# flyakon/DeepPhysiNet

Hardware: AMD Instinct MI355X
Metric: collocation-points/sec (fwd+PDE-Jacobian+bwd) (higher is better)
Workload: dtype bf16x2 (hi+lo split bf16 MFMA operands), fp32 accumulate

## Files before the change

deepphysinet_amd/csrc/dpn_device.h:

```cpp
#pragma once
#include <hip/hip_runtime.h>
#include <stdint.h>
#include <stdio.h>
#include <stdlib.h>

#include "../../include/dpn_hip.h"
#include "dpn_layout.h"

using namespace dpn;

typedef __attribute__((ext_vector_type(8))) __bf16 bf16x8;
typedef __attribute__((ext_vector_type(16))) float f32x16;
typedef unsigned short u16;

#define DEV __device__ __forceinline__

typedef unsigned int u32;
typedef __attribute__((ext_vector_type(2))) __bf16 bf16x2;
typedef __attribute__((ext_vector_type(2))) float f32x2;
typedef __attribute__((ext_vector_type(4))) u32 u32x4;
typedef __attribute__((ext_vector_type(4))) float f32x4;

DEV u32 pack2(float a, float b) {
    const f32x2 v = {a, b};
    return __builtin_bit_cast(u32, __builtin_convertvector(v, bf16x2));
}
DEV float bf_lo(u32 w) { return __uint_as_float(w << 16); }
DEV float bf_hi(u32 w) { return __uint_as_float(w & 0xFFFF0000u); }

DEV bf16x8 as_bf(u32x4 w) { return __builtin_bit_cast(bf16x8, w); }
DEV f32x16 mfma(bf16x8 a, bf16x8 b, f32x16 c) { return __builtin_amdgcn_mfma_f32_32x32x16_bf16(a, b, c, 0, 0, 0); }

static inline int ck(hipError_t e) { return (int)e; }
```

deepphysinet_amd/csrc/dpn_encoder_chain.hip:

```cpp
#include <atomic>
#include <hip/hip_runtime.h>
#include <stdint.h>
#include <stdlib.h>

#include "../../include/dpn_hip.h"
#include "../../include/dpn_hip_experiments.h"

#define DEV __device__ __forceinline__

namespace {

typedef _Float16 f16x8 __attribute__((ext_vector_type(8)));
typedef float f32x4 __attribute__((ext_vector_type(4)));
typedef unsigned int u32;
typedef u32 u32x4 __attribute__((ext_vector_type(4)));

constexpr int kD = 256;
constexpr int kThreads = 512, kWaves = 8;
constexpr int kImgBytes = 256 * 1024;
#ifndef DPN_ENC_PF
#define DPN_ENC_PF 8
#endif
template <int NTT> constexpr int pf_of() { return NTT == 1 ? DPN_ENC_PF : 4; }
constexpr int kYS = 260;
constexpr int kXImg = 16384;
constexpr float kLoScale = 2048.0f, kLoInv = 1.0f / 2048.0f;

#ifdef DPN_ENC_TIMELINE
unsigned* g_enc_timeline = nullptr;
#define ENC_STAMP(I) do { if (a.tl && lane == 0) a.tl[((size_t)tl_block * kWaves + wave) * 32 + (I)] = (unsigned)__builtin_readcyclecounter(); } while (0)
#define ENC_TL_ARG unsigned* tl;
#define ENC_TL_SET(A) (A).tl = g_enc_timeline
#else
#define ENC_STAMP(I) do { } while (0)
#define ENC_TL_ARG
#define ENC_TL_SET(A) do { } while (0)
#endif

DEV void barrier_lds() {
    __builtin_amdgcn_fence(__ATOMIC_RELEASE, "workgroup", "local");
    __builtin_amdgcn_s_barrier();
    __builtin_amdgcn_fence(__ATOMIC_ACQUIRE, "workgroup", "local");
}

template <int CTRL>
DEV float dpp(float v) { return __builtin_bit_cast(float, __builtin_amdgcn_update_dpp(0, __builtin_bit_cast(int, v), CTRL, 0xf, 0xf, false)); }
DEV float swz16(float v) { return __builtin_bit_cast(float, __builtin_amdgcn_ds_swizzle(__builtin_bit_cast(int, v), 0x401F)); }
DEV float half_sum(float v) {
    v += dpp<0xB1>(v);
    v += dpp<0x4E>(v);
    v += dpp<0x141>(v);
    v += dpp<0x140>(v);
    v += swz16(v);
    return v;
}
DEV float half_max(float v) {
    v = fmaxf(v, dpp<0xB1>(v));
    v = fmaxf(v, dpp<0x4E>(v));
    v = fmaxf(v, dpp<0x141>(v));
    v = fmaxf(v, dpp<0x140>(v));
    v = fmaxf(v, swz16(v));
    return v;
}

DEV float gelu_exact(float x) { return x * 0.5f * (1.0f + erff(x * 0.70710678118654752440f)); }
DEV float gelu_exact_grad(float x) {
    const float cdf = 0.5f * (1.0f + erff(x * 0.70710678118654752440f));
    const float pdf = expf(-0.5f * x * x) * 0.39894228040143267794f;
    return cdf + x * pdf;
}

DEV void split8(const float (&v)[8], u32x4& hi, u32x4& lo) {
    f16x8 h, l;
#pragma unroll
    for (int e = 0; e < 8; ++e) {
        const _Float16 a = (_Float16)v[e];
        h[e] = a;
        l[e] = (_Float16)((v[e] - (float)a) * kLoScale);
    }
    hi = __builtin_bit_cast(u32x4, h);
    lo = __builtin_bit_cast(u32x4, l);
}

DEV int xpos(int slot, int n) { return slot * 16 + (n ^ ((slot & 3) | ((slot & 4) ? 12 : 0))); }

struct RowLane {
    int tsel, slot, n16;
    DEV RowLane(int wave, int lane) : tsel(lane >> 5), slot(lane & 31), n16(2 * wave + (lane >> 5)) {}
};

DEV void row_to_ximg(const float (&v)[8], const float extra_max, const RowLane& rl, char* ximg_tile, float* rscale_tile) {
    float m = extra_max;
#pragma unroll
    for (int e = 0; e < 8; ++e) m = fmaxf(m, fabsf(v[e]));
    m = half_max(m);
    int eb = (__builtin_bit_cast(int, m) >> 23) & 0xff;
    eb = eb < 4 ? 4 : eb;
    const float sc = __builtin_bit_cast(float, (257 - eb) << 23);
    float s[8];
#pragma unroll
    for (int e = 0; e < 8; ++e) s[e] = v[e] * sc;
    u32x4 hi, lo;
    split8(s, hi, lo);
    char* p = ximg_tile + xpos(rl.slot, rl.n16) * 16;
    *reinterpret_cast<u32x4*>(p) = hi;
    *reinterpret_cast<u32x4*>(p + kXImg / 2) = lo;
    if (rl.slot == 0) rscale_tile[rl.n16] = __builtin_bit_cast(float, (eb - 3) << 23);
}
DEV float row_absmax(const float (&v)[8]) {
    float m = 0.f;
#pragma unroll
    for (int e = 0; e < 8; ++e) m = fmaxf(m, fabsf(v[e]));
    return m;
}

DEV void load8(float (&v)[8], const float* p, bool ok) {
    if (ok) {
        const float4 a = reinterpret_cast<const float4*>(p)[0], b = reinterpret_cast<const float4*>(p)[1];
        v[0] = a.x; v[1] = a.y; v[2] = a.z; v[3] = a.w; v[4] = b.x; v[5] = b.y; v[6] = b.z; v[7] = b.w;
    } else {
#pragma unroll
        for (int e = 0; e < 8; ++e) v[e] = 0.f;
    }
}
DEV void store8(float* p, const float (&v)[8], bool ok) {
    if (ok) {
        reinterpret_cast<float4*>(p)[0] = make_float4(v[0], v[1], v[2], v[3]);
        reinterpret_cast<float4*>(p)[1] = make_float4(v[4], v[5], v[6], v[7]);
    }
}
DEV void lds8(float (&v)[8], const float* p) {
    const f32x4 a = reinterpret_cast<const f32x4*>(p)[0], b = reinterpret_cast<const f32x4*>(p)[1];
    v[0] = a[0]; v[1] = a[1]; v[2] = a[2]; v[3] = a[3]; v[4] = b[0]; v[5] = b[1]; v[6] = b[2]; v[7] = b[3];
}

DEV void layer_norm8(const float (&v)[8], const float (&gam)[8], const float (&bet)[8], float (&xhat)[8], float (&y)[8], float& rstd) {
    float s = 0.f;
#pragma unroll
    for (int e = 0; e < 8; ++e) s += v[e];
    const float mean = half_sum(s) * (1.f / kD);
    float d[8], q = 0.f;
#pragma unroll
    for (int e = 0; e < 8; ++e) { d[e] = v[e] - mean; q = fmaf(d[e], d[e], q); }
    rstd = 1.0f / sqrtf(half_sum(q) * (1.f / kD) + 1e-5f);
#pragma unroll
    for (int e = 0; e < 8; ++e) { xhat[e] = d[e] * rstd; y[e] = fmaf(xhat[e], gam[e], bet[e]); }
}
DEV void layer_norm_bwd8(const float (&g)[8], const float (&xhat)[8], const float rstd, const float (&gam)[8], float (&gx)[8], float (&pg)[8],
                         float (&pb)[8]) {
    float t[8], s1 = 0.f, s2 = 0.f;
#pragma unroll
    for (int e = 0; e < 8; ++e) { t[e] = g[e] * gam[e]; s1 += t[e]; s2 = fmaf(t[e], xhat[e], s2); pg[e] = fmaf(g[e], xhat[e], pg[e]); pb[e] += g[e]; }
    const float m1 = half_sum(s1) * (1.f / kD), m2 = half_sum(s2) * (1.f / kD);
#pragma unroll
    for (int e = 0; e < 8; ++e) gx[e] = rstd * (t[e] - m1 - xhat[e] * m2);
}

struct WStream {
    __amdgpu_buffer_rsrc_t rs;
    int voff, tile_off;
    DEV void init(const void* wpack, int64_t bytes, int wave, int lane) {
        rs = __builtin_amdgcn_make_buffer_rsrc(const_cast<void*>(wpack), 0, (int)bytes, 0x00020000);
        voff = lane * 16;
        tile_off = wave * 2 * 16384;
    }
    template <int NT>
    DEV void load(u32x4 (&dst)[NT][2], int img_off, int ks) const {
#pragma unroll
        for (int t = 0; t < NT; ++t)
#pragma unroll
            for (int p = 0; p < 2; ++p)
                dst[t][p] = __builtin_bit_cast(u32x4, __builtin_amdgcn_raw_buffer_load_b128(rs, voff + p * 1024, img_off + tile_off + t * 16384 + ks * 2048, 0));
    }
};
template <int PF, int NT = 2> struct Ring { u32x4 a[PF][NT][2]; };

DEV f32x4 mfma(u32x4 a, u32x4 b, f32x4 c) {
    return __builtin_amdgcn_mfma_f32_16x16x32_f16(__builtin_bit_cast(f16x8, a), __builtin_bit_cast(f16x8, b), c, 0, 0, 0);
}

template <int NTT, int NT = 2>
struct Acc {
    f32x4 m[NT][NTT], c[NT][NTT];
    DEV void zero() {
#pragma unroll
        for (int t = 0; t < NT; ++t)
#pragma unroll
            for (int tt = 0; tt < NTT; ++tt) { m[t][tt] = (f32x4)0.f; c[t][tt] = (f32x4)0.f; }
    }
};

template <int NTT, bool HAS_NEXT, int NT = 2>
DEV void gemm(const WStream& ws, Ring<pf_of<NTT>(), NT>& R, const int cur_off, const int next_off, const char* xr0, const char* xr1, Acc<NTT, NT>& acc) {
    u32x4 B[2][NTT][2];
    auto loadB = [&](const int ks, const int buf) __attribute__((always_inline)) {
        const char* base = ((ks & 1) ? xr1 : xr0) + ks * 1024;
// ... 1320 lines not shown
```

deepphysinet_amd/csrc/dpn_fwd_tiles.h:

```cpp
#pragma once

namespace ts {
constexpr int kVecFloats = kNumVecs * 256 + 4;
template <int NS>
struct Cfg {
    static constexpr int kXBytes = 16 * 2 * NS * 1024;
    static constexpr int kVecOff = kXBytes;
    static constexpr int kRedOff = kVecOff + kVecFloats * 4;
    static constexpr int kLdsBytes = kRedOff + 4 * 64 * 4;
};

DEV void barrier_lds() {
    __builtin_amdgcn_fence(__ATOMIC_RELEASE, "workgroup", "local");
    __builtin_amdgcn_s_barrier();
    __builtin_amdgcn_fence(__ATOMIC_ACQUIRE, "workgroup", "local");
}

struct NoSide { DEV void operator()(int) const {} };

#ifdef TS_ABL_NOSINCOS
template <int NS> DEV void ts_sincos(float th, float& s, float& c) { s = th; c = th * 0.5f; }
#else
template <int NS> DEV void ts_sincos(float th, float& s, float& c) { sincos_t<NS>(th, s, c); }
#endif

template <int NS, bool SWAP = false>
DEV void mma3(const u32x4 (&a)[NS], const u32x4 (&b)[NS], f32x16& acc) {
#ifdef TS_ABL_NOMFMA
    if constexpr (NS == 2) asm volatile("" ::"v"(a[0]), "v"(a[1]), "v"(b[0]), "v"(b[1]));
    else asm volatile("" ::"v"(a[0]), "v"(b[0]));
    return;
#endif
    if constexpr (SWAP) {
        if constexpr (NS == 2) {
            acc = mfma(as_bf(b[1]), as_bf(a[0]), acc);
            acc = mfma(as_bf(b[0]), as_bf(a[1]), acc);
        }
        acc = mfma(as_bf(b[0]), as_bf(a[0]), acc);
    } else {
        if constexpr (NS == 2) {
            acc = mfma(as_bf(a[0]), as_bf(b[1]), acc);
            acc = mfma(as_bf(a[1]), as_bf(b[0]), acc);
        }
        acc = mfma(as_bf(a[0]), as_bf(b[0]), acc);
    }
}

#ifndef TS_PF
#define TS_PF 3
#endif
#ifndef TS_PRIO
#define TS_PRIO 2
#endif
#ifndef TS_DEFER_SAVES
#define TS_DEFER_SAVES 1
#endif
#ifndef TS_SCHED_GROUPS
#define TS_SCHED_GROUPS 0
#endif
constexpr int kPF = TS_PF;
template <int NS, int NT> struct Head { u32x4 a[kPF - 1][NT][NS]; };

template <int NS, int NK, int NT>
struct WSrc {
    __amdgpu_buffer_rsrc_t rs;
    int voff;
    int so[NT];
    DEV void init(const char* wg, const int lane, const int ks0) {
        rs = __builtin_amdgcn_make_buffer_rsrc(const_cast<char*>(wg), 0, NT * NK * NS * 1024, 0x00020000);
        voff = lane * 16;
#pragma unroll
        for (int t = 0; t < NT; ++t) { so[t] = (t * NK + ks0) * NS * 1024; asm volatile("" : "+s"(so[t])); }
    }
    DEV void next(u32x4 (&dst)[NT][NS]) {
#pragma unroll
        for (int t = 0; t < NT; ++t) {
#pragma unroll
            for (int s = 0; s < NS; ++s) {
#ifdef TS_ABL_NOALOAD
                asm volatile("" : "=v"(dst[t][s]));
#else
                dst[t][s] = __builtin_bit_cast(u32x4, __builtin_amdgcn_raw_buffer_load_b128(rs, voff + s * 1024, so[t], 0));
#endif
            }
            so[t] += NS * 1024;
            asm volatile("" : "+s"(so[t]));
        }
    }
};
template <int NS, int NK, int NT>
DEV void gemm_head(const char* wg, const int lane, Head<NS, NT>& H) {
    WSrc<NS, NK, NT> src;
    src.init(wg, lane, 0);
#pragma unroll
    for (int k = 0; k < kPF - 1; ++k) src.next(H.a[k]);
}
template <int NS, int NK, int NT, bool SWAP = false, class Side = NoSide, bool PIN = true, bool SG = PIN>
DEV void gemm(const char* wg, const char* xl, const int lane, const Head<NS, NT>& H, f32x16 (&acc)[2][2], const Side& side = Side()) {
    static_assert(NK >= kPF, "k-steps per chunk");
    WSrc<NS, NK, NT> src;
    src.init(wg, lane, kPF - 1);
    u32x4 A[kPF][NT][NS];
    u32x4 B[2][2][NS];
    auto loadB = [&](const int ks, const int slot) __attribute__((always_inline)) {
#pragma unroll
        for (int p = 0; p < 2; ++p)
#pragma unroll
            for (int s = 0; s < NS; ++s) B[slot][p][s] = *reinterpret_cast<const u32x4*>(xl + ((ks * 2 + p) * NS + s) * 1024);
    };
#pragma unroll
    for (int k = 0; k < kPF - 1; ++k)
#pragma unroll
        for (int t = 0; t < NT; ++t)
#pragma unroll
            for (int s = 0; s < NS; ++s) A[k][t][s] = H.a[k][t][s];
    loadB(0, 0);
#if TS_PRIO == 2
    __builtin_amdgcn_s_setprio(0);
#endif
#pragma unroll
    for (int ks = 0; ks < NK; ++ks) {
        if (ks + kPF - 1 < NK) src.next(A[(ks + kPF - 1) % kPF]);
        if (ks + 1 < NK) loadB(ks + 1, (ks + 1) & 1);
#if TS_SCHED_GROUPS
        if (SG && ks + 1 < NK) {
            __builtin_amdgcn_sched_group_barrier(0x100, 2 * NS, 0);
            __builtin_amdgcn_sched_group_barrier(0x008, 4 * (NS == 2 ? 3 : 1), 0);
        }
#endif
#if TS_PRIO == 1
        __builtin_amdgcn_s_setprio(1);
#endif
#pragma unroll
        for (int t = 0; t < NT; ++t)
#pragma unroll
            for (int p = 0; p < 2; ++p) mma3<NS, SWAP>(A[ks % kPF][t], B[ks & 1][p], acc[t][p]);
#if TS_PRIO == 1
        __builtin_amdgcn_s_setprio(0);
#endif
        side(ks);
        if constexpr (PIN) {
        asm volatile("" : "+v"(acc[0][0]), "+v"(acc[0][1]), "+v"(acc[1][0]), "+v"(acc[1][1]));
        }
    }
#if TS_PRIO == 2
    __builtin_amdgcn_s_setprio(1);
#endif
}

template <int NS>
DEV void x_store(char* xl, const int ks, const int p, const Frag<NS>& f) {
#pragma unroll
    for (int s = 0; s < NS; ++s) *reinterpret_cast<u32x4*>(xl + ((ks * 2 + p) * NS + s) * 1024) = f.w[s];
}

DEV void acc_init(f32x16& acc, const float* vec, const int which, const int h, const int T, const float scale) {
    const f32x4* v = reinterpret_cast<const f32x4*>(vec + which * 256 + h * 128 + T * 16);
#pragma unroll
    for (int q = 0; q < 4; ++q) {
        const f32x4 x = v[q];
        acc[4 * q] = scale * x[0]; acc[4 * q + 1] = scale * x[1]; acc[4 * q + 2] = scale * x[2]; acc[4 * q + 3] = scale * x[3];
    }
}

struct Ident { u32x4 a, b; };
DEV Ident make_ident(const int j, const int h) {
    Ident I;
    const int mine = (((j >> 3) & 1) == h) ? (j & 7) : -1;
#pragma unroll
// ... 138 lines not shown
```

deepphysinet_amd/csrc/dpn_gemm.hip:

```cpp
#include "dpn_device.h"

struct SgemmArgs {
    const float *A, *B, *bias;
    float *C, *asum, *ws;
    int M, N, K, lda, ldb, ldc, ta, tb, accumulate, k_per_split;
};

__global__ __launch_bounds__(256) void dpn_sgemm_kernel(SgemmArgs a) {
    constexpr int BM = 32, BN = 32, BK = 32;
    __shared__ float As[BK][BM + 1];
    __shared__ float Bs[BK][BN + 1];
    const int tx = threadIdx.x & 15, ty = threadIdx.x >> 4;
    const int m0 = blockIdx.y * BM, n0 = blockIdx.x * BN;
    const int kbeg = blockIdx.z * a.k_per_split;
    const int kend = (kbeg + a.k_per_split < a.K) ? kbeg + a.k_per_split : a.K;
    const bool split = gridDim.z > 1;
    float acc[2][2] = {{0.f, 0.f}, {0.f, 0.f}};
    float rs = 0.f;
    const bool do_asum = a.asum != nullptr && blockIdx.x == 0;
    float ra[4], rb[4];
    auto gload = [&](int k0) __attribute__((always_inline)) {
#pragma unroll
        for (int i = 0; i < 4; ++i) {
            const int e = threadIdx.x + 256 * i;
            {
                const int kk = a.ta ? (e >> 5) : (e & 31), mm = a.ta ? (e & 31) : (e >> 5);
                const int gm = m0 + mm, gk = k0 + kk;
                ra[i] = (gm < a.M && gk < kend) ? (a.ta ? a.A[(int64_t)gk * a.lda + gm] : a.A[(int64_t)gm * a.lda + gk]) : 0.f;
            }
            {
                const int kk = a.tb ? (e & 31) : (e >> 5), nn = a.tb ? (e >> 5) : (e & 31);
                const int gk = k0 + kk, gn = n0 + nn;
                rb[i] = (gk < kend && gn < a.N) ? (a.tb ? a.B[(int64_t)gn * a.ldb + gk] : a.B[(int64_t)gk * a.ldb + gn]) : 0.f;
            }
        }
    };
    gload(kbeg);
    for (int k0 = kbeg; k0 < kend; k0 += BK) {
#pragma unroll
        for (int i = 0; i < 4; ++i) {
            const int e = threadIdx.x + 256 * i;
            As[a.ta ? (e >> 5) : (e & 31)][a.ta ? (e & 31) : (e >> 5)] = ra[i];
            Bs[a.tb ? (e & 31) : (e >> 5)][a.tb ? (e >> 5) : (e & 31)] = rb[i];
        }
        __syncthreads();
        if (k0 + BK < kend) gload(k0 + BK);
#pragma unroll
        for (int kk = 0; kk < BK; ++kk) {
            const float a0 = As[kk][ty], a1 = As[kk][ty + 16], b0 = Bs[kk][tx], b1 = Bs[kk][tx + 16];
            acc[0][0] = fmaf(a0, b0, acc[0][0]); acc[0][1] = fmaf(a0, b1, acc[0][1]);
            acc[1][0] = fmaf(a1, b0, acc[1][0]); acc[1][1] = fmaf(a1, b1, acc[1][1]);
        }
        if (do_asum && threadIdx.x < BM) {
#pragma unroll
            for (int kk = 0; kk < BK; ++kk) rs += As[kk][threadIdx.x];
        }
        __syncthreads();
    }
#pragma unroll
    for (int i = 0; i < 2; ++i)
#pragma unroll
        for (int j = 0; j < 2; ++j) {
            const int gm = m0 + ty + 16 * i, gn = n0 + tx + 16 * j;
            if (gm < a.M && gn < a.N) {
                if (split) {
                    a.ws[((int64_t)blockIdx.z * a.M + gm) * a.N + gn] = acc[i][j];
                } else {
                    const float v = acc[i][j] + (a.bias ? a.bias[gn] : 0.f);
                    float* c = a.C + (int64_t)gm * a.ldc + gn;
                    *c = a.accumulate ? (*c + v) : v;
                }
            }
        }
    if (do_asum && threadIdx.x < BM && m0 + threadIdx.x < a.M) {
        if (split) a.ws[(int64_t)gridDim.z * a.M * a.N + (int64_t)blockIdx.z * a.M + m0 + threadIdx.x] = rs;
        else a.asum[m0 + threadIdx.x] = rs;
    }
}

__global__ __launch_bounds__(256) void dpn_sgemm_reduce_kernel(SgemmArgs a, int splits) {
    const int64_t idx = (int64_t)blockIdx.x * 256 + threadIdx.x;
    const int64_t mn = (int64_t)a.M * a.N;
    if (idx < mn) {
        float v = 0.f;
        for (int z = 0; z < splits; ++z) v += a.ws[z * mn + idx];
        const int gm = (int)(idx / a.N), gn = (int)(idx % a.N);
        v += a.bias ? a.bias[gn] : 0.f;
        float* c = a.C + (int64_t)gm * a.ldc + gn;
        *c = a.accumulate ? (*c + v) : v;
    }
    if (a.asum && idx < a.M) {
        float v = 0.f;
        for (int z = 0; z < splits; ++z) v += a.ws[splits * mn + (int64_t)z * a.M + idx];
        a.asum[idx] = v;
    }
}

constexpr int kBatchMaxProblems = DPN_GEMM_MAX_PROBLEMS, kBatchMaxTerms = DPN_GEMM_MAX_TERMS, kBatchTermPool = 32, kBatchMaxJobs = DPN_GEMM_MAX_JOBS;
struct SgemmTerm {
    const float* A;
    const float* B;
    int lda, ldb, K, pad;
};
struct SgemmProblem {
    const float* bias;
    float *C, *asum;
    const float* aux;
    float* aux_out;
    int M, N, ldc, ta, tb, nterms, term0, epi;
};
DEV float gelu_exact(float x) { return x * 0.5f * (1.0f + erff(x * 0.70710678118654752440f)); }
DEV float gelu_exact_grad(float x) {
    const float cdf = 0.5f * (1.0f + erff(x * 0.70710678118654752440f));
    const float pdf = expf(-0.5f * x * x) * 0.39894228040143267794f;
    return cdf + x * pdf;
}
struct SgemmColsum { const float* partial; float* out_a; float* out_b; int nblocks, pad; };
struct SgemmBatch {
    SgemmProblem p[kBatchMaxProblems];
    SgemmTerm t[kBatchTermPool];
    SgemmColsum job[kBatchMaxJobs];
    int n;
};

typedef float f32x1;
DEV f32x16 mfma_f32(float a, float b, f32x16 c) { return __builtin_amdgcn_mfma_f32_32x32x2f32(a, b, c, 0, 0, 0); }

template <int BK, int NBUF, int NT = 256, int TM = 1, int TN = 1>
__global__ __launch_bounds__(NT) void dpn_sgemm_batch_kernel(SgemmBatch batch) {
    constexpr int BM = 32 * TM, BN = 32 * TN, NLA = BK * BM / NT, NLB = BK * BN / NT;
    constexpr int NW = NT / 64, NQ = TM * TN, KW = NW / NQ;
    static_assert(NW % NQ == 0 && BK % (2 * KW) == 0 && (BK * BM) % NT == 0 && (BK * BN) % NT == 0, "tile shape");
    const int bx = blockIdx.x, by = blockIdx.y, bz = blockIdx.z;
    if (bz >= batch.n) {
        if (bx || by) return;
        const SgemmColsum& j = batch.job[bz - batch.n];
        const int c = threadIdx.x;
        if (c >= 256) return;
        float s1 = 0.f, s2 = 0.f;
#pragma unroll 8
        for (int b = 0; b < j.nblocks; ++b) { s1 += j.partial[(int64_t)b * 512 + c]; s2 += j.partial[(int64_t)b * 512 + 256 + c]; }
        j.out_a[c] = s1;
        j.out_b[c] = s2;
        return;
    }
    const SgemmProblem& a = batch.p[bz];
    const int m0 = by * BM, n0 = bx * BN;
    if (m0 >= a.M || n0 >= a.N) return;
    struct Stage { float A[NBUF][BK][BM + 1]; float B[NBUF][BK][BN + 1]; };
    __shared__ Stage stage;
    float (&As)[NBUF][BK][BM + 1] = stage.A;
    float (&Bs)[NBUF][BK][BN + 1] = stage.B;
    float (*part)[32 * 33] = reinterpret_cast<float (*)[32 * 33]>(&stage);
    const int wave_q = (threadIdx.x >> 6) % NQ, wave_k = (threadIdx.x >> 6) / NQ, qm = wave_q / TN, qn = wave_q % TN;
    static_assert(sizeof(Stage) >= NW * 32 * 33 * sizeof(float), "partial tiles must fit in the staging buffers");
    const int lane = threadIdx.x & 63, wave = threadIdx.x >> 6;
    const int i = lane & 31, h = lane >> 5;
    f32x16 acc = (f32x16)0.f;
    float rs = 0.f;
    const bool do_asum = a.asum != nullptr && bx == 0;
    int total = 0;
    for (int t = 0; t < a.nterms; ++t) total += (batch.t[a.term0 + t].K + BK - 1) / BK;
    const int ktiles0 = (batch.t[a.term0].K + BK - 1) / BK;
    float ra[NLA], rb[NLB];
    int lt = 0, lk0 = 0;
    auto gload = [&]() __attribute__((always_inline)) {
        const SgemmTerm& T = batch.t[a.term0 + lt];
        const float* A = T.A;
        const float* B = T.B;
        const int lda = T.lda, ldb = T.ldb, K = T.K, k0 = lk0;
#pragma unroll
        for (int q = 0; q < NLA; ++q) {
            const int e = threadIdx.x + NT * q;
            const int kk = a.ta ? (e / BM) : (e % BK), mm = a.ta ? (e % BM) : (e / BK);
            const int gm = m0 + mm, gk = k0 + kk;
            ra[q] = (gm < a.M && gk < K) ? (a.ta ? A[(int64_t)gk * lda + gm] : A[(int64_t)gm * lda + gk]) : 0.f;
        }
#pragma unroll
        for (int q = 0; q < NLB; ++q) {
            const int e = threadIdx.x + NT * q;
            const int kk = a.tb ? (e % BK) : (e / BN), nn = a.tb ? (e / BK) : (e % BN);
            const int gk = k0 + kk, gn = n0 + nn;
            rb[q] = (gk < K && gn < a.N) ? (a.tb ? B[(int64_t)gn * ldb + gk] : B[(int64_t)gk * ldb + gn]) : 0.f;
        }
        lk0 += BK;
        if (lk0 >= K) { lk0 = 0; ++lt; }
    };
    auto lstore = [&](int buf) __attribute__((always_inline)) {
#pragma unroll
        for (int q = 0; q < NLA; ++q) {
            const int e = threadIdx.x + NT * q;
            As[buf][a.ta ? (e / BM) : (e % BK)][a.ta ? (e % BM) : (e / BK)] = ra[q];
        }
#pragma unroll
        for (int q = 0; q < NLB; ++q) {
            const int e = threadIdx.x + NT * q;
            Bs[buf][a.tb ? (e % BK) : (e / BN)][a.tb ? (e / BK) : (e % BN)] = rb[q];
        }
    };
    if constexpr (NBUF == 2) {
        gload();
        lstore(0);
        if (total > 1) gload();
        __syncthreads();
        for (int it = 0; it < total; ++it) {
            const int buf = it & 1;
            if (it + 1 < total) lstore(buf ^ 1);
            if (it + 2 < total) gload();
#pragma unroll
            for (int u = 0; u < BK / (2 * KW); ++u) {
                const int kk = wave_k * (BK / KW) + 2 * u + h;
                acc = mfma_f32(As[buf][kk][32 * qm + i], Bs[buf][kk][32 * qn + i], acc);
            }
            if (do_asum && it < ktiles0 && threadIdx.x < BM) {
#pragma unroll
                for (int kk = 0; kk < BK; ++kk) rs += As[buf][kk][threadIdx.x];
            }
            __syncthreads();
        }
    } else {
        gload();
        for (int it = 0; it < total; ++it) {
            lstore(0);
            __syncthreads();
            if (it + 1 < total) gload();
#pragma unroll 8
            for (int u = 0; u < BK / (2 * KW); ++u) {
                const int kk = wave_k * (BK / KW) + 2 * u + h;
                acc = mfma_f32(As[0][kk][32 * qm + i], Bs[0][kk][32 * qn + i], acc);
            }
            if (do_asum && it < ktiles0 && threadIdx.x < BM) {
#pragma unroll 8
                for (int kk = 0; kk < BK; ++kk) rs += As[0][kk][threadIdx.x];
            }
            __syncthreads();
        }
    }
#pragma unroll
    for (int r = 0; r < 16; ++r) part[wave][drow32(r, h) * 33 + i] = acc[r];
    __syncthreads();
#pragma unroll
    for (int e = threadIdx.x; e < 1024 * NQ; e += NT) {
        const int sq = e >> 10, r = (e >> 5) & 31, c = e & 31, o = r * 33 + c;
        const int gr = m0 + 32 * (sq / TN) + r, gc = n0 + 32 * (sq % TN) + c;
        if (gr < a.M && gc < a.N) {
            float v = part[sq][o];
#pragma unroll
            for (int w_ = 1; w_ < KW; ++w_) v += part[w_ * NQ + sq][o];
            v += a.bias ? a.bias[gc] : 0.f;
            const int64_t idx = (int64_t)gr * a.ldc + gc;
            if (a.epi == DPN_EPI_GELU) { if (a.aux_out) a.aux_out[idx] = v; v = gelu_exact(v); }
            else if (a.epi == DPN_EPI_MUL_GELU_GRAD) v *= gelu_exact_grad(a.aux[idx]);
            else if (a.epi == DPN_EPI_ADD) v += a.aux[idx];
            a.C[idx] = v;
        }
    }
    if (do_asum && threadIdx.x < BM && m0 + threadIdx.x < a.M) a.asum[m0 + threadIdx.x] = rs;
}

struct LnGemmArgs {
    int mode, M, N, tb, ldb, ldc, epi;
    const float *x, *r, *gamma, *beta, *rstd_in;
    float *y_out, *xhat_out, *rstd_out, *partial;
    const float *B, *bias;
    float* C;
    const float* aux;
    float* aux_out;
};
template <int MODE, int NT = 512>
__global__ __launch_bounds__(NT) void dpn_sgemm_ln_kernel(LnGemmArgs a) {
    constexpr int BK = 256;
    constexpr int NW = NT / 64;
    constexpr int TPR = NT / 32, CW = 256 / TPR;
    __shared__ float As[BK][33];
    __shared__ float Bs[BK][33];
    const int t = threadIdx.x, lane = t & 63, wave = t >> 6, i = lane & 31, h = lane >> 5;
    const int m0 = blockIdx.y * 32, n0 = blockIdx.x * 32;
    const bool keep = blockIdx.x == 0;
    constexpr int NLB = BK * 32 / NT;
    float rb[NLB];
#pragma unroll
    for (int q = 0; q < NLB; ++q) {
        const int e = t + NT * q;
        const int kk = a.tb ? (e & 255) : (e >> 5), nn = a.tb ? (e >> 8) : (e & 31);
        const int gn = n0 + nn;
        rb[q] = (gn < a.N) ? (a.tb ? a.B[(int64_t)gn * a.ldb + kk] : a.B[(int64_t)kk * a.ldb + gn]) : 0.f;
    }
    const int m = t / TPR, c0 = (t % TPR) * CW, gm = m0 + m;
    const bool ok = gm < a.M;
    float v[CW], w[MODE == 2 ? CW : 1], gam[CW];
#pragma unroll
    for (int j = 0; j < CW / 4; ++j) {
        const float4 x4 = ok ? *reinterpret_cast<const float4*>(a.x + (int64_t)gm * 256 + c0 + 4 * j) : make_float4(0.f, 0.f, 0.f, 0.f);
        const float4 g4 = *reinterpret_cast<const float4*>(a.gamma + c0 + 4 * j);
        v[4 * j] = x4.x; v[4 * j + 1] = x4.y; v[4 * j + 2] = x4.z; v[4 * j + 3] = x4.w;
        gam[4 * j] = g4.x; gam[4 * j + 1] = g4.y; gam[4 * j + 2] = g4.z; gam[4 * j + 3] = g4.w;
        if (MODE == 1) {
            if (ok && a.r) {
                const float4 r4 = *reinterpret_cast<const float4*>(a.r + (int64_t)gm * 256 + c0 + 4 * j);
                v[4 * j] += r4.x; v[4 * j + 1] += r4.y; v[4 * j + 2] += r4.z; v[4 * j + 3] += r4.w;
            }
        } else {
            const float4 r4 = ok ? *reinterpret_cast<const float4*>(a.r + (int64_t)gm * 256 + c0 + 4 * j) : make_float4(0.f, 0.f, 0.f, 0.f);
            w[4 * j] = r4.x; w[4 * j + 1] = r4.y; w[4 * j + 2] = r4.z; w[4 * j + 3] = r4.w;
        }
    }
    auto row_sum = [&](float s_) __attribute__((always_inline)) {
        s_ += __shfl_xor(s_, 1); s_ += __shfl_xor(s_, 2); s_ += __shfl_xor(s_, 4);
        if constexpr (TPR == 16) s_ += __shfl_xor(s_, 8);
        return s_;
    };
    if (MODE == 2 && keep) {
#pragma unroll
        for (int j = 0; j < CW; ++j) { As[c0 + j][m] = v[j]; Bs[c0 + j][m] = w[j]; }
        __syncthreads();
        if (t < 256) {
            float dg = 0.f, db = 0.f;
#pragma unroll 8
            for (int q = 0; q < 32; ++q) { dg = fmaf(As[t][q], Bs[t][q], dg); db += As[t][q]; }
            a.partial[(int64_t)blockIdx.y * 512 + t] = dg;
            a.partial[(int64_t)blockIdx.y * 512 + 256 + t] = db;
        }
        __syncthreads();
    }
    if (MODE == 1) {
        float s_ = 0.f;
#pragma unroll
        for (int j = 0; j < CW; ++j) s_ += v[j];
        const float mean = row_sum(s_) * (1.f / 256.f);
        float q_ = 0.f;
#pragma unroll
        for (int j = 0; j < CW; ++j) { const float d = v[j] - mean; q_ = fmaf(d, d, q_); }
        const float rstd = 1.0f / sqrtf(row_sum(q_) * (1.f / 256.f) + 1e-5f);
        if (keep && ok && (t % TPR) == 0) a.rstd_out[gm] = rstd;
#pragma unroll
        for (int j = 0; j < CW / 4; ++j) {
            const float4 b4 = *reinterpret_cast<const float4*>(a.beta + c0 + 4 * j);
            const float bb[4] = {b4.x, b4.y, b4.z, b4.w};
            float xh[4], yy[4];
#pragma unroll
            for (int e = 0; e < 4; ++e) { xh[e] = (v[4 * j + e] - mean) * rstd; yy[e] = fmaf(xh[e], gam[4 * j + e], bb[e]); v[4 * j + e] = yy[e]; }
            if (keep && ok) {
                *reinterpret_cast<float4*>(a.xhat_out + (int64_t)gm * 256 + c0 + 4 * j) = make_float4(xh[0], xh[1], xh[2], xh[3]);
                *reinterpret_cast<float4*>(a.y_out + (int64_t)gm * 256 + c0 + 4 * j) = make_float4(yy[0], yy[1], yy[2], yy[3]);
            }
        }
    } else {
        float s1 = 0.f, s2 = 0.f;
#pragma unroll
        for (int j = 0; j < CW; ++j) { const float tk = v[j] * gam[j]; s1 += tk; s2 = fmaf(tk, w[j], s2); }
        const float m1 = row_sum(s1) * (1.f / 256.f), m2 = row_sum(s2) * (1.f / 256.f);
        const float rs_ = ok ? a.rstd_in[gm] : 0.f;
#pragma unroll
        for (int j = 0; j < CW / 4; ++j) {
#pragma unroll
            for (int e = 0; e < 4; ++e) v[4 * j + e] = rs_ * (v[4 * j + e] * gam[4 * j + e] - m1 - w[4 * j + e] * m2);
            if (keep && ok) *reinterpret_cast<float4*>(a.y_out + (int64_t)gm * 256 + c0 + 4 * j) = make_float4(v[4 * j], v[4 * j + 1], v[4 * j + 2], v[4 * j + 3]);
        }
    }
#pragma unroll
    for (int j = 0; j < CW; ++j) As[c0 + j][m] = v[j];
#pragma unroll
    for (int q = 0; q < NLB; ++q) {
        const int e = t + NT * q;
        Bs[a.tb ? (e & 255) : (e >> 5)][a.tb ? (e >> 8) : (e & 31)] = rb[q];
    }
    __syncthreads();
    f32x16 acc = (f32x16)0.f;
#pragma unroll 8
    for (int u = 0; u < BK / (2 * NW); ++u) {
        const int kk = wave * (BK / NW) + 2 * u + h;
        acc = mfma_f32(As[kk][i], Bs[kk][i], acc);
    }
    __syncthreads();
    float (*partt)[32 * 33] = reinterpret_cast<float (*)[32 * 33]>(&As[0][0]);
#pragma unroll
    for (int r = 0; r < 16; ++r) partt[wave][drow32(r, h) * 33 + i] = acc[r];
    __syncthreads();
#pragma unroll
    for (int e = t; e < 1024; e += NT) {
        const int r = e >> 5, c = e & 31, o = r * 33 + c;
        if (m0 + r < a.M && n0 + c < a.N) {
            float vv = partt[0][o];
#pragma unroll
            for (int w_ = 1; w_ < NW; ++w_) vv += partt[w_][o];
            vv += a.bias ? a.bias[n0 + c] : 0.f;
            const int64_t idx = (int64_t)(m0 + r) * a.ldc + n0 + c;
            if (a.epi == DPN_EPI_GELU) { if (a.aux_out) a.aux_out[idx] = vv; vv = gelu_exact(vv); }
            else if (a.epi == DPN_EPI_MUL_GELU_GRAD) vv *= gelu_exact_grad(a.aux[idx]);
            else if (a.epi == DPN_EPI_ADD) vv += a.aux[idx];
            a.C[idx] = vv;
        }
    }
}

extern "C" {

int dpn_sgemm(int ta, int tb, int M, int N, int K, const float* A, int lda, const float* B, int ldb, float* C, int ldc,
              const float* bias, float* asum, int accumulate, void* workspace, int64_t workspace_bytes, void* stream) {
    if (!A || !B || !C || M <= 0 || N <= 0 || K <= 0) return -1;
    hipStream_t s = reinterpret_cast<hipStream_t>(stream);
    const int tiles = ((N + 31) / 32) * ((M + 31) / 32);
    int splits = 1;
    if (workspace && tiles < 256 && K >= 1024) {
        splits = (512 + tiles - 1) / tiles;
        const int maxs = K / 256;
        if (splits > maxs) splits = maxs;
        if (splits > 32) splits = 32;
        while (splits > 1 && (int64_t)splits * ((int64_t)M * N + M) * 4 > workspace_bytes) --splits;
        if (splits < 1) splits = 1;
    }
    int kps = (K + splits - 1) / splits;
    kps = ((kps + 31) / 32) * 32;
    splits = (K + kps - 1) / kps;
    SgemmArgs a{A, B, bias, C, asum, reinterpret_cast<float*>(workspace), M, N, K, lda, ldb, ldc, ta, tb, accumulate, kps};
    hipLaunchKernelGGL(dpn_sgemm_kernel, dim3((N + 31) / 32, (M + 31) / 32, splits), dim3(256), 0, s, a);
    if (splits > 1) {
        const int64_t work = (int64_t)M * N > M ? (int64_t)M * N : M;
        hipLaunchKernelGGL(dpn_sgemm_reduce_kernel, dim3((unsigned)((work + 255) / 256)), dim3(256), 0, s, a, splits);
    }
    return ck(hipGetLastError());
}

constexpr int kSingleStageMaxTiles = 1;
constexpr long kSingleStageMaxOutTiles = 512;
static int sgemm_batch_launch(int n_problems, const DpnGemmProblem* problems, int n_jobs, const DpnColsumJob* jobs, void* stream) {
    if (n_problems <= 0 || n_problems > kBatchMaxProblems || !problems || n_jobs < 0 || n_jobs > kBatchMaxJobs || (n_jobs && !jobs)) return -1;
    static_assert(sizeof(SgemmBatch) <= 4096, "kernel arguments");
    SgemmBatch b;
    b.n = n_problems;
    int gx = 0, gy = 0, pool = 0;
    for (int i = 0; i < n_problems; ++i) {
        const DpnGemmProblem& q = problems[i];
        if (q.nterms < 1 || q.nterms > kBatchMaxTerms || pool + q.nterms > kBatchTermPool || !q.C || q.M <= 0 || q.N <= 0) return -1;
        if (q.epi < 0 || q.epi > DPN_EPI_ADD || ((q.epi == DPN_EPI_MUL_GELU_GRAD || q.epi == DPN_EPI_ADD) && !q.aux)) return -1;
        if (q.asum && q.nterms != 1) return -1;
        SgemmProblem& p = b.p[i];
        p.term0 = pool;
        for (int t = 0; t < q.nterms; ++t) {
            const int kt = q.k_term[t] > 0 ? q.k_term[t] : q.K;
            if (!q.A[t] || !q.B[t] || kt <= 0) return -1;
            b.t[pool++] = SgemmTerm{q.A[t], q.B[t], q.lda[t], q.ldb[t], kt, 0};
        }
        p.bias = q.bias; p.C = q.C; p.asum = q.asum; p.aux = q.aux; p.aux_out = q.aux_out; p.epi = q.epi;
        p.M = q.M; p.N = q.N; p.ldc = q.ldc; p.ta = q.ta; p.tb = q.tb; p.nterms = q.nterms;
        gx = gx > (q.N + 31) / 32 ? gx : (q.N + 31) / 32;
        gy = gy > (q.M + 31) / 32 ? gy : (q.M + 31) / 32;
    }
    for (int i = 0; i < n_jobs; ++i) {
        if (!jobs[i].partial || !jobs[i].out_a || !jobs[i].out_b || jobs[i].n_blocks <= 0) return -1;
        b.job[i] = SgemmColsum{jobs[i].partial, jobs[i].out_a, jobs[i].out_b, jobs[i].n_blocks, 0};
    }
    const int gz = n_problems + n_jobs;
    bool single_tile = true;
    long out_tiles = 0;
    for (int i = 0; i < n_problems; ++i) {
        int tiles = 0;
        for (int t = 0; t < b.p[i].nterms; ++t) tiles += (b.t[b.p[i].term0 + t].K + 255) / 256;
        single_tile = single_tile && tiles <= kSingleStageMaxTiles;
        out_tiles += (long)((b.p[i].M + 31) / 32) * ((b.p[i].N + 31) / 32);
    }
    single_tile = single_tile && out_tiles <= kSingleStageMaxOutTiles;
    if (single_tile) {
        hipLaunchKernelGGL((dpn_sgemm_batch_kernel<256, 1, 512>), dim3(gx, gy, gz), dim3(512), 0, reinterpret_cast<hipStream_t>(stream), b);
        return ck(hipGetLastError());
    }
    hipLaunchKernelGGL((dpn_sgemm_batch_kernel<64, 2, 512>), dim3(gx, gy, gz), dim3(512), 0, reinterpret_cast<hipStream_t>(stream), b);
    return ck(hipGetLastError());
}

int dpn_sgemm_batch(int n_problems, const DpnGemmProblem* problems, void* stream) {
    return sgemm_batch_launch(n_problems, problems, 0, nullptr, stream);
}

int dpn_sgemm_batch_jobs(int n_problems, const DpnGemmProblem* problems, int n_jobs, const DpnColsumJob* jobs, void* stream) {
    return sgemm_batch_launch(n_problems, problems, n_jobs, jobs, stream);
}

int dpn_sgemm_ln(const DpnLnGemm* q, void* stream) {
    if (!q || (q->mode != 1 && q->mode != 2) || q->M <= 0 || q->N <= 0 || !q->x || !q->gamma || !q->B || !q->C || !q->y_out) return -1;
    if (q->mode == 1 && (!q->beta || !q->xhat_out || !q->rstd_out)) return -1;
    if (q->mode == 2 && (!q->r || !q->rstd_in || !q->partial)) return -1;
    if (q->epi < 0 || q->epi > DPN_EPI_ADD || ((q->epi == DPN_EPI_MUL_GELU_GRAD || q->epi == DPN_EPI_ADD) && !q->aux)) return -1;
    LnGemmArgs a{q->mode, q->M, q->N, q->tb, q->ldb, q->ldc, q->epi, q->x, q->r, q->gamma, q->beta, q->rstd_in, q->y_out, q->xhat_out,
                 q->rstd_out, q->partial, q->B, q->bias, q->C, q->aux, q->aux_out};
    const dim3 grid((q->N + 31) / 32, (q->M + 31) / 32);
    if (q->mode == 1) hipLaunchKernelGGL((dpn_sgemm_ln_kernel<1, 512>), grid, dim3(512), 0, reinterpret_cast<hipStream_t>(stream), a);
    else hipLaunchKernelGGL((dpn_sgemm_ln_kernel<2, 512>), grid, dim3(512), 0, reinterpret_cast<hipStream_t>(stream), a);
    return ck(hipGetLastError());
}

}
```

Baseline: 35.70 million.

## Add deeper register-ring prefetch pipeline with buffer loads to batched sgemm

Adds a ring-buffered main loop for the multi-tile fp32 batched GEMM. It keeps several K-tiles of global loads in flight in registers (depth 3 by default) using raw buffer loads with out-of-bounds clamping, and crosses multi-term boundaries without draining the pipeline. It also sets a waves-per-EU occupancy hint on the pipelined kernel and moves the barrier helper into a shared header. The trade is higher register pressure in exchange for hiding global memory latency. The buffer offsets must stay under 2GB, so the host falls back to the old loop when an operand is too large.

```diff
diff --git a/deepphysinet_amd/csrc/dpn_barrier.h b/deepphysinet_amd/csrc/dpn_barrier.h
--- /dev/null
+++ b/deepphysinet_amd/csrc/dpn_barrier.h
@@ -0,0 +1,8 @@
+#pragma once
+#include <hip/hip_runtime.h>
+
+__device__ __forceinline__ void barrier_lds() {
+    __builtin_amdgcn_fence(__ATOMIC_RELEASE, "workgroup", "local");
+    __builtin_amdgcn_s_barrier();
+    __builtin_amdgcn_fence(__ATOMIC_ACQUIRE, "workgroup", "local");
+}
diff --git a/deepphysinet_amd/csrc/dpn_device.h b/deepphysinet_amd/csrc/dpn_device.h
--- a/deepphysinet_amd/csrc/dpn_device.h
+++ b/deepphysinet_amd/csrc/dpn_device.h
@@ -5,6 +5,7 @@
 #include <stdlib.h>
 
 #include "../../include/dpn_hip.h"
+#include "dpn_barrier.h"
 #include "dpn_layout.h"
 
 using namespace dpn;
diff --git a/deepphysinet_amd/csrc/dpn_encoder_chain.hip b/deepphysinet_amd/csrc/dpn_encoder_chain.hip
--- a/deepphysinet_amd/csrc/dpn_encoder_chain.hip
+++ b/deepphysinet_amd/csrc/dpn_encoder_chain.hip
@@ -5,6 +5,7 @@
 
 #include "../../include/dpn_hip.h"
 #include "../../include/dpn_hip_experiments.h"
+#include "dpn_barrier.h"
 
 #define DEV __device__ __forceinline__
 
@@ -36,12 +37,6 @@
 #define ENC_TL_ARG
 #define ENC_TL_SET(A) do { } while (0)
 #endif
-
-DEV void barrier_lds() {
-    __builtin_amdgcn_fence(__ATOMIC_RELEASE, "workgroup", "local");
-    __builtin_amdgcn_s_barrier();
-    __builtin_amdgcn_fence(__ATOMIC_ACQUIRE, "workgroup", "local");
-}
 
 template <int CTRL>
 DEV float dpp(float v) { return __builtin_bit_cast(float, __builtin_amdgcn_update_dpp(0, __builtin_bit_cast(int, v), CTRL, 0xf, 0xf, false)); }
diff --git a/deepphysinet_amd/csrc/dpn_fwd_tiles.h b/deepphysinet_amd/csrc/dpn_fwd_tiles.h
--- a/deepphysinet_amd/csrc/dpn_fwd_tiles.h
+++ b/deepphysinet_amd/csrc/dpn_fwd_tiles.h
@@ -10,11 +10,7 @@
     static constexpr int kLdsBytes = kRedOff + 4 * 64 * 4;
 };
 
-DEV void barrier_lds() {
-    __builtin_amdgcn_fence(__ATOMIC_RELEASE, "workgroup", "local");
-    __builtin_amdgcn_s_barrier();
-    __builtin_amdgcn_fence(__ATOMIC_ACQUIRE, "workgroup", "local");
-}
+using ::barrier_lds;
 
 struct NoSide { DEV void operator()(int) const {} };
 
diff --git a/deepphysinet_amd/csrc/dpn_gemm.hip b/deepphysinet_amd/csrc/dpn_gemm.hip
--- a/deepphysinet_amd/csrc/dpn_gemm.hip
+++ b/deepphysinet_amd/csrc/dpn_gemm.hip
@@ -108,6 +108,7 @@
     const float* aux;
     float* aux_out;
     int M, N, ldc, ta, tb, nterms, term0, epi;
+    int tiles64, ktiles0_64, ring, pad;
 };
 DEV float gelu_exact(float x) { return x * 0.5f * (1.0f + erff(x * 0.70710678118654752440f)); }
 DEV float gelu_exact_grad(float x) {
@@ -126,8 +127,138 @@
 typedef float f32x1;
 DEV f32x16 mfma_f32(float a, float b, f32x16 c) { return __builtin_amdgcn_mfma_f32_32x32x2f32(a, b, c, 0, 0, 0); }
 
+#ifndef DPN_SGEMM_DEPTH
+#define DPN_SGEMM_DEPTH 3
+#endif
+#ifndef DPN_SGEMM_SKIP_TAIL
+#define DPN_SGEMM_SKIP_TAIL 0
+#endif
+#ifndef DPN_SGEMM_WAVES
+#define DPN_SGEMM_WAVES 8
+#endif
+constexpr int kPipeDepth = DPN_SGEMM_DEPTH;
+constexpr int kOutsideOffset = 0x7ffffff0;
+constexpr int64_t kRingMaxBytes = (1ll << 31) - 64;
+
+#ifdef DPN_SGEMM_TIMELINE
+__device__ unsigned* g_sgemm_tl = nullptr;
+constexpr int kTlSlots = 16, kTlLast = kTlSlots - 1;
+#define SG_STAMP(I) do { if (g_sgemm_tl && (threadIdx.x & 63) == 0 && (I) < kTlSlots) \
+    g_sgemm_tl[((((size_t)blockIdx.z * gridDim.y + blockIdx.y) * gridDim.x + blockIdx.x) * 8 + (threadIdx.x >> 6)) * kTlSlots + (I)] = (unsigned)__builtin_readcyclecounter(); } while (0)
+#else
+#define SG_STAMP(I) do { } while (0)
+#endif
+
+template <int BK, int NT, int TM, int TN>
+DEV void sgemm_ring_loop(const SgemmBatch& batch, const SgemmProblem& a, float* As, float* Bs, const int m0, const int n0, const bool do_asum,
+                         f32x16& acc, float& rs) {
+    constexpr int D = kPipeDepth, BM = 32 * TM, BN = 32 * TN, NLA = BK * BM / NT, NLB = BK * BN / NT, SA = BM + 1, SB = BN + 1;
+    constexpr int NW = NT / 64, NQ = TM * TN, KW = NW / NQ, KPW = BK / KW;
+    static_assert(NT % BM == 0 && NT % BN == 0 && NT % BK == 0 && D >= 1, "ring loads");
+    const int tid = threadIdx.x, lane = tid & 63, i = lane & 31, h = lane >> 5;
+    const int wave = __builtin_amdgcn_readfirstlane(tid >> 6), wave_q = wave % NQ, wave_k = wave / NQ, qm = wave_q / TN, qn = wave_q % TN;
+    const int M = a.M, N = a.N, nterms = a.nterms, term0 = a.term0, total = a.tiles64, ktiles0 = a.ktiles0_64;
+    const bool ta = a.ta != 0, tb = a.tb != 0;
+    const int ak = ta ? tid / BM : tid % BK, am = ta ? tid % BM : tid / BK;
+    const int bk = tb ? tid % BK : tid / BN, bn = tb ? tid / BK : tid % BN;
+    const int aq = ta ? NT / BM : NT / BK, bq = tb ? NT / BK : NT / BN;
+    float* const a_st = As + ak * SA + am;
+    float* const b_st = Bs + bk * SB + bn;
+    const int a_sq = ta ? aq * SA : aq, b_sq = tb ? bq : bq * SB;
+    const float* const a_ld = As + (wave_k * KPW + h) * SA + 32 * qm + i;
+    const float* const b_ld = Bs + (wave_k * KPW + h) * SB + 32 * qn + i;
+    __amdgpu_buffer_rsrc_t rsa, rsb;
+    int voa = 0, vob = 0, qa = 0, qb = 0;
+    int lt = 0, lk0 = 0, kcur = 0, soa = 0, sob = 0, stepa = 0, stepb = 0;
+    SgemmTerm nxt = batch.t[term0];
+    auto enter_term = [&]() __attribute__((always_inline)) {
+        const float *A = nxt.A, *B = nxt.B;
+        const int lda = nxt.lda, ldb = nxt.ldb, K = nxt.K;
+        nxt = batch.t[term0 + (lt + 1 < nterms ? lt + 1 : lt)];
+        rsa = __builtin_amdgcn_make_buffer_rsrc(const_cast<float*>(A), 0, (ta ? (K - 1) * lda + M : (M - 1) * lda + K) * 4, 0x00020000);
+        rsb = __builtin_amdgcn_make_buffer_rsrc(const_cast<float*>(B), 0, (tb ? (N - 1) * ldb + K : (K - 1) * ldb + N) * 4, 0x00020000);
+        voa = ta ? (m0 + am < M ? (ak * lda + m0 + am) * 4 : kOutsideOffset) : ((m0 + am) * lda + ak) * 4;
+        vob = tb ? ((n0 + bn) * ldb + bk) * 4 : (n0 + bn < N ? (bk * ldb + n0 + bn) * 4 : kOutsideOffset);
+        qa = aq * lda * 4; qb = bq * ldb * 4;
+        kcur = K; lk0 = 0; soa = 0; sob = 0;
+        stepa = (ta ? lda * BK : BK) * 4;
+        stepb = (tb ? BK : ldb * BK) * 4;
+    };
+    auto fetch = [&](float (&da)[NLA], float (&db)[NLB], int& kv) __attribute__((always_inline)) {
+#pragma unroll
+        for (int q = 0; q < NLA; ++q) da[q] = __builtin_bit_cast(float, __builtin_amdgcn_raw_buffer_load_b32(rsa, voa + q * qa, soa, 0));
+#pragma unroll
+        for (int q = 0; q < NLB; ++q) db[q] = __builtin_bit_cast(float, __builtin_amdgcn_raw_buffer_load_b32(rsb, vob + q * qb, sob, 0));
+        kv = kcur - lk0;
+        lk0 += BK; soa += stepa; sob += stepb;
+        if (lk0 >= kcur) {
+            if (++lt < nterms) {
+                enter_term();
+            } else {
+                rsa = __builtin_amdgcn_make_buffer_rsrc(nullptr, 0, 0, 0x00020000);
+                rsb = rsa;
+                kcur = 0x7fffffff; lk0 = 0; soa = 0; sob = 0; stepa = 0; stepb = 0; qa = 0; qb = 0;
+            }
+        }
+    };
+    auto to_lds = [&](const float (&da)[NLA], const float (&db)[NLB], const int kv, const int stage) __attribute__((always_inline)) {
+        const bool in_k = (tid % BK) < kv;
+        const bool keep_a = ta || in_k, keep_b = !tb || in_k;
+        float* pa = a_st + stage * (BK * SA);
+        float* pb = b_st + stage * (BK * SB);
+#pragma unroll
+        for (int q = 0; q < NLA; ++q) pa[q * a_sq] = keep_a ? da[q] : 0.f;
+#pragma unroll
+        for (int q = 0; q < NLB; ++q) pb[q * b_sq] = keep_b ? db[q] : 0.f;
+    };
+    auto compute = [&](const int stage, const int kv, const int it) __attribute__((always_inline)) {
+        const float* pa = a_ld + stage * (BK * SA);
+        const float* pb = b_ld + stage * (BK * SB);
+#pragma unroll
+        for (int u = 0; u < KPW / 2; ++u) {
+            if (DPN_SGEMM_SKIP_TAIL && wave_k * KPW + 2 * u >= kv) break;
+            acc = mfma_f32(pa[2 * u * SA], pb[2 * u * SB], acc);
+        }
+        if (do_asum && it < ktiles0 && tid < BM) {
+            const float* ps = As + stage * (BK * SA) + tid;
+#pragma unroll 32
+            for (int kk = 0; kk < BK; ++kk) rs += ps[kk * SA];
+        }
+    };
+    float ra[D][NLA], rb[D][NLB];
+    int kv[D];
+    enter_term();
+#pragma unroll
+    for (int d = 0; d < D; ++d) fetch(ra[d], rb[d], kv[d]);
+    SG_STAMP(0);
+    int kv_cur = kv[0], stage = 0, it = 0;
+    to_lds(ra[0], rb[0], kv_cur, 0);
+    SG_STAMP(1);
+    fetch(ra[0], rb[0], kv[0]);
+    barrier_lds();
+    while (it + 1 < total) {
+#pragma unroll
+        for (int d = 0; d < D; ++d) {
+            const int s = (d + 1) % D;
+            const bool live = it + 1 < total;
+            const int kv_next = kv[s];
+            if (live) to_lds(ra[s], rb[s], kv_next, stage ^ 1);
+            fetch(ra[s], rb[s], kv[s]);
+            if (live) {
+                compute(stage, kv_cur, it);
+                barrier_lds();
+                SG_STAMP(2 + it < kTlLast ? 2 + it : kTlLast - 1);
+                kv_cur = kv_next; stage ^= 1; ++it;
+            }
+        }
+    }
+    compute(stage, kv_cur, it);
+    SG_STAMP(2 + it < kTlLast ? 2 + it : kTlLast - 1);
+    __syncthreads();
+}
+
 template <int BK, int NBUF, int NT = 256, int TM = 1, int TN = 1>
-__global__ __launch_bounds__(NT) void dpn_sgemm_batch_kernel(SgemmBatch batch) {
+__global__ __launch_bounds__(NT) __attribute__((amdgpu_waves_per_eu(NBUF == 2 ? DPN_SGEMM_WAVES : 2))) void dpn_sgemm_batch_kernel(SgemmBatch batch) {
     constexpr int BM = 32 * TM, BN = 32 * TN, NLA = BK * BM / NT, NLB = BK * BN / NT;
     constexpr int NW = NT / 64, NQ = TM * TN, KW = NW / NQ;
     static_assert(NW % NQ == 0 && BK % (2 * KW) == 0 && (BK * BM) % NT == 0 && (BK * BN) % NT == 0, "tile shape");
@@ -199,6 +330,11 @@
         }
     };
     if constexpr (NBUF == 2) {
+      if (a.ring) {
+        float* const as0 = &As[0][0][0];
+        float* const bs0 = &Bs[0][0][0];
+        sgemm_ring_loop<BK, NT, TM, TN>(batch, a, as0, bs0, m0, n0, do_asum, acc, rs);
+      } else {
         gload();
         lstore(0);
         if (total > 1) gload();
@@ -218,6 +354,7 @@
             }
             __syncthreads();
         }
+      }
     } else {
         gload();
         for (int it = 0; it < total; ++it) {
@@ -256,6 +393,7 @@
         }
     }
     if (do_asum && threadIdx.x < BM && m0 + threadIdx.x < a.M) a.asum[m0 + threadIdx.x] = rs;
+    if constexpr (NBUF == 2) SG_STAMP(kTlLast);
 }
 
 struct LnGemmArgs {
@@ -422,14 +560,18 @@
     return ck(hipGetLastError());
 }
 
+enum { DPN_SGEMM_FORM_SINGLE_STAGE = 1, DPN_SGEMM_FORM_PIPELINED = 2, DPN_SGEMM_FORM_PIPELINED_GENERIC = 3 };
 constexpr int kSingleStageMaxTiles = 1;
 constexpr long kSingleStageMaxOutTiles = 512;
-static int sgemm_batch_launch(int n_problems, const DpnGemmProblem* problems, int n_jobs, const DpnColsumJob* jobs, void* stream) {
+static bool ring_operand(int64_t rows, int64_t cols, int64_t ld) {
+    return ld >= cols && ((rows + 64) * ld + cols + 64) * 4 < kRingMaxBytes;
+}
+static int sgemm_batch_plan(int n_problems, const DpnGemmProblem* problems, int n_jobs, const DpnColsumJob* jobs, SgemmBatch& b, dim3& grid) {
     if (n_problems <= 0 || n_problems > kBatchMaxProblems || !problems || n_jobs < 0 || n_jobs > kBatchMaxJobs || (n_jobs && !jobs)) return -1;
     static_assert(sizeof(SgemmBatch) <= 4096, "kernel arguments");
-    SgemmBatch b;
     b.n = n_problems;
     int gx = 0, gy = 0, pool = 0;
+    bool all_ring = true;
     for (int i = 0; i < n_problems; ++i) {
         const DpnGemmProblem& q = problems[i];
         if (q.nterms < 1 || q.nterms > kBatchMaxTerms || pool + q.nterms > kBatchTermPool || !q.C || q.M <= 0 || q.N <= 0) return -1;
@@ -437,11 +579,23 @@
         if (q.asum && q.nterms != 1) return -1;
         SgemmProblem& p = b.p[i];
         p.term0 = pool;
+        p.tiles64 = 0;
+        bool ring = true;
         for (int t = 0; t < q.nterms; ++t) {
             const int kt = q.k_term[t] > 0 ? q.k_term[t] : q.K;
             if (!q.A[t] || !q.B[t] || kt <= 0) return -1;
             b.t[pool++] = SgemmTerm{q.A[t], q.B[t], q.lda[t], q.ldb[t], kt, 0};
-        }
+            p.tiles64 += (kt + 63) / 64;
+            if (t == 0) p.ktiles0_64 = (kt + 63) / 64;
+            ring = ring && (q.ta ? ring_operand(kt, q.M, q.lda[t]) : ring_operand(q.M, kt, q.lda[t]))
+                        && (q.tb ? ring_operand(q.N, kt, q.ldb[t]) : ring_operand(kt, q.N, q.ldb[t]));
+        }
+#ifdef DPN_SGEMM_FORCE_GENERIC
+        ring = false;
+#endif
+        p.ring = ring ? 1 : 0;
+        p.pad = 0;
+        all_ring = all_ring && ring;
         p.bias = q.bias; p.C = q.C; p.asum = q.asum; p.aux = q.aux; p.aux_out = q.aux_out; p.epi = q.epi;
         p.M = q.M; p.N = q.N; p.ldc = q.ldc; p.ta = q.ta; p.tb = q.tb; p.nterms = q.nterms;
         gx = gx > (q.N + 31) / 32 ? gx : (q.N + 31) / 32;
@@ -451,7 +605,7 @@
         if (!jobs[i].partial || !jobs[i].out_a || !jobs[i].out_b || jobs[i].n_blocks <= 0) return -1;
         b.job[i] = SgemmColsum{jobs[i].partial, jobs[i].out_a, jobs[i].out_b, jobs[i].n_blocks, 0};
     }
-    const int gz = n_problems + n_jobs;
+    grid = dim3(gx, gy, n_problems + n_jobs);
     bool single_tile = true;
     long out_tiles = 0;
     for (int i = 0; i < n_problems; ++i) {
@@ -461,13 +615,31 @@
         out_tiles += (long)((b.p[i].M + 31) / 32) * ((b.p[i].N + 31) / 32);
     }
     single_tile = single_tile && out_tiles <= kSingleStageMaxOutTiles;
-    if (single_tile) {
-        hipLaunchKernelGGL((dpn_sgemm_batch_kernel<256, 1, 512>), dim3(gx, gy, gz), dim3(512), 0, reinterpret_cast<hipStream_t>(stream), b);
+    return single_tile ? DPN_SGEMM_FORM_SINGLE_STAGE : all_ring ? DPN_SGEMM_FORM_PIPELINED : DPN_SGEMM_FORM_PIPELINED_GENERIC;
+}
+
+static int sgemm_batch_launch(int n_problems, const DpnGemmProblem* problems, int n_jobs, const DpnColsumJob* jobs, void* stream) {
+    SgemmBatch b;
+    dim3 grid;
+    const int form = sgemm_batch_plan(n_problems, problems, n_jobs, jobs, b, grid);
+    if (form < 0) return -1;
+    if (form == DPN_SGEMM_FORM_SINGLE_STAGE) {
+        hipLaunchKernelGGL((dpn_sgemm_batch_kernel<256, 1, 512>), grid, dim3(512), 0, reinterpret_cast<hipStream_t>(stream), b);
         return ck(hipGetLastError());
     }
-    hipLaunchKernelGGL((dpn_sgemm_batch_kernel<64, 2, 512>), dim3(gx, gy, gz), dim3(512), 0, reinterpret_cast<hipStream_t>(stream), b);
+    hipLaunchKernelGGL((dpn_sgemm_batch_kernel<64, 2, 512>), grid, dim3(512), 0, reinterpret_cast<hipStream_t>(stream), b);
     return ck(hipGetLastError());
 }
+
+int dpn_sgemm_batch_form(int n_problems, const DpnGemmProblem* problems, int n_jobs, const DpnColsumJob* jobs) {
+    SgemmBatch b;
+    dim3 grid;
+    return sgemm_batch_plan(n_problems, problems, n_jobs, jobs, b, grid);
+}
+
+#ifdef DPN_SGEMM_TIMELINE
+int dpn_sgemm_debug_set_timeline(unsigned* stamps) { return ck(hipMemcpyToSymbol(HIP_SYMBOL(g_sgemm_tl), &stamps, sizeof(stamps))); }
+#endif
 
 int dpn_sgemm_batch(int n_problems, const DpnGemmProblem* problems, void* stream) {
     return sgemm_batch_launch(n_problems, problems, 0, nullptr, stream);
```

After: 35.79 million, median of 6. No clear change (+0.2%).
